# ikryukov/svo

Hardware: AMD Instinct MI355X
Metric: frames/sec @1241x376, 2000 feats; LK iters/sec; achieved HBM GB/s (higher is better)
Workload: dtype u8/int32 fixed-point (LK sums exact int, solve f32), f64 PnP

## Files before the change

svo_amd/csrc/lk_device.hpp:

```cpp
#pragma once
#include "common.hpp"

#include <cfloat>
#include <cmath>

namespace svo {

namespace {

constexpr int W_BITS = 14;
constexpr float FLT_SCALE = 1.f / (1 << 20);
constexpr int JM = 3;

struct LKDev {
    int win_w, win_h, groups;
    int ip_w, ip_h, jr_w, jr_h;
    int ip_bytes, lds_wave;
    int max_level, max_count;
    double eps2;
    float eps2_lo, eps2_hi;
    int flags, want_err;
    float min_eig;
};

inline LKDev lk_dev(const LKParams& lp) {
    LKDev d;
    d.win_w = lp.win_w;
    d.win_h = lp.win_h;
    d.groups = 64 / lp.win_w;
    d.ip_w = lp.win_w;
    d.ip_h = lp.win_h + 1;
    d.jr_w = lp.win_w + 2 * JM;
    d.jr_h = lp.win_h + 1 + 2 * JM;
    d.ip_bytes = (d.ip_w * d.ip_h * 4 + 15) & ~15;
    d.lds_wave = d.ip_bytes + ((d.jr_w * d.jr_h * 4 + 15) & ~15);
    d.max_level = lp.max_level;
    d.max_count = lp.max_count;
    d.eps2 = lp.eps2;
    d.eps2_lo = (float)(lp.eps2 * (1.0 - 0x1p-20));
    d.eps2_hi = (float)(lp.eps2 * (1.0 + 0x1p-20));
    if ((double)d.eps2_lo > lp.eps2 * (1.0 - 0x1p-20)) d.eps2_lo = nextafterf(d.eps2_lo, 0.f);
    if ((double)d.eps2_hi < lp.eps2 * (1.0 + 0x1p-20)) d.eps2_hi = nextafterf(d.eps2_hi, INFINITY);
    d.flags = lp.flags;
    d.want_err = lp.want_err;
    d.min_eig = lp.min_eig;
    return d;
}

__device__ __forceinline__ bool converged(float dx, float dy, float lo, float hi, double eps2) {
    const float sf = dx * dx + dy * dy;
    bool c = sf < lo;
    if (__builtin_expect(sf >= lo && sf <= hi, 0)) {
        asm volatile("" ::: "memory");
        c = (double)dx * dx + (double)dy * dy <= eps2;
    }
    return c;
}
__device__ __forceinline__ bool below_001(float v) { return fabsf(v) <= 0x1.47ae14p-7f; }

__device__ __forceinline__ int refl101(int p, int len) {
    if ((unsigned)p < (unsigned)len) return p;
    if (len == 1) return 0;
    do {
        p = p < 0 ? -p : 2 * len - 2 - p;
    } while ((unsigned)p >= (unsigned)len);
    return p;
}

__device__ __forceinline__ int ufloor(float v) {
    return (int)__builtin_floorf(v);
}
__device__ __forceinline__ float uni_f(float v) {
    return __int_as_float(__builtin_amdgcn_readfirstlane(__float_as_int(v)));
}
__device__ __forceinline__ int uni_i(int v) { return __builtin_amdgcn_readfirstlane(v); }

__device__ __forceinline__ void wave_lds_sync() {
    __builtin_amdgcn_fence(__ATOMIC_SEQ_CST, "wavefront");
    __builtin_amdgcn_wave_barrier();
}

__device__ __forceinline__ int dpp_sum(int v) {
    v += __builtin_amdgcn_update_dpp(0, v, 0xb1, 0xf, 0xf, true);
    v += __builtin_amdgcn_update_dpp(0, v, 0x4e, 0xf, 0xf, true);
    v += __builtin_amdgcn_update_dpp(0, v, 0x114, 0xf, 0xf, true);
    v += __builtin_amdgcn_update_dpp(0, v, 0x118, 0xf, 0xf, true);
    v += __builtin_amdgcn_update_dpp(0, v, 0x142, 0xa, 0xf, true);
    v += __builtin_amdgcn_update_dpp(0, v, 0x143, 0xc, 0xf, true);
    return __builtin_amdgcn_readlane(v, 63);
}
__device__ __forceinline__ double wave_sum_exact(int v) {
    int hi = dpp_sum(v >> 16);
    int lo = dpp_sum(v & 0xFFFF);
    return (double)((long long)hi * 65536 + (long long)lo);
}
template <int CTRL, int ROW_MASK, bool BC>
__device__ __forceinline__ int dpp_add(int v) {
    return v + __builtin_amdgcn_update_dpp(0, v, CTRL, ROW_MASK, 0xf, BC);
}

typedef const __attribute__((address_space(1))) uint8_t* gu8;
typedef const __attribute__((address_space(1))) uint32_t* gu32;
typedef short s16x2 __attribute__((ext_vector_type(2)));
typedef uint32_t u32x2a4 __attribute__((ext_vector_type(2), aligned(4)));
typedef uint16_t u16a1 __attribute__((aligned(1)));
typedef const __attribute__((address_space(4))) PyrDesc* cpyr;

template <typename T>
__device__ __forceinline__ T ldg_off(gu8 base, unsigned off) {
    return *(const __attribute__((address_space(1))) T*)(base + off);
}
__device__ __forceinline__ gu8 pad_origin(const uint8_t* data, int pitch, int pad_px, int elem) {
    return (gu8)data - (size_t)pad_px * ((size_t)pitch + 1) * elem;
}

__device__ __forceinline__ int sdot2(unsigned a, unsigned b, int c) {
    return __builtin_amdgcn_sdot2(__builtin_bit_cast(s16x2, a), __builtin_bit_cast(s16x2, b), c, false);
}
__device__ __forceinline__ int sdot2_r(unsigned a, unsigned b, int c) {
    int d;
    asm("v_dot2_i32_i16 %0, %1, %2, %3" : "=v"(d) : "v"(a), "v"(b), "v"(c));
    return d;
}
__device__ __forceinline__ unsigned lo16x2(int lo, int hi) {
    return __builtin_amdgcn_perm((unsigned)hi, (unsigned)lo, 0x05040100u);
}

__device__ __forceinline__ unsigned wbits(float p) { return __float_as_uint(p + 768.f); }
struct BiW {
    unsigned W0, W1;
};
__device__ __forceinline__ BiW bilinear_weights(float a, float b) {
    const float ia = 1.f - a, ib = 1.f - b;
    const unsigned b00 = wbits(ia * ib), b01 = wbits(a * ib), b10 = wbits(ia * b);
    const unsigned w11 = (1u << W_BITS) + 3u * 0x44400000u - b00 - b01 - b10;
    return {__builtin_amdgcn_perm(b01, b00, 0x05040100u), __builtin_amdgcn_perm(w11, b10, 0x05040100u)};
}

struct SubPix {
    int ix, iy;
    BiW w;
};
__device__ __forceinline__ SubPix sub_pixel(float x, float y) {
    const float fx = __builtin_floorf(x), fy = __builtin_floorf(y);
    return {(int)fx, (int)fy, bilinear_weights(x - fx, y - fy)};
}
__device__ __forceinline__ bool window_in_bounds(int x, int y, int w, int h, int win_w, int win_h) {
    return (unsigned)(x + win_w) < (unsigned)(w + win_w) && (unsigned)(y + win_h) < (unsigned)(h + win_h);
}

struct LevelStart {
    float nextx, nexty;
    int ipx, ipy;
    bool inb;
    float a, b;
};
__device__ __forceinline__ LevelStart level_start(float px, float py, float nx, float ny, int level, int max_level,
                                                  int flags, int lw, int lh, int win_w, int win_h) {
    const float halfWx = (win_w - 1) * 0.5f, halfWy = (win_h - 1) * 0.5f;
    const float lscale = __builtin_amdgcn_ldexpf(1.f, -level);
    float prevx = px * lscale, prevy = py * lscale;
    float nextx, nexty;
    if (level == max_level) {
        if (flags & SVO_LK_USE_INITIAL_FLOW) {
            nextx = nx * lscale;
            nexty = ny * lscale;
        } else {
            nextx = prevx;
            nexty = prevy;
        }
    } else {
        nextx = nx * 2.f;
        nexty = ny * 2.f;
    }
    prevx -= halfWx;
    prevy -= halfWy;
    const float fpx = __builtin_floorf(prevx), fpy = __builtin_floorf(prevy);
    const int ipx = (int)fpx, ipy = (int)fpy;
    return {nextx, nexty, ipx, ipy, window_in_bounds(ipx, ipy, lw, lh, win_w, win_h), prevx - fpx, prevy - fpy};
}

template <int M, class Stage>
__device__ __forceinline__ void follow_region(int x, int y, int& jx0, int& jy0, Stage stage) {
    if ((unsigned)(x - jx0) > 2u * M || (unsigned)(y - jy0) > 2u * M) {
        jx0 = x - M;
        jy0 = y - M;
        wave_lds_sync();
        stage();
        wave_lds_sync();
    }
}

template <int M, class Stage, class RowSad>
__device__ __forceinline__ bool sad_error(float nx, float ny, int jw, int jh, int win_w, int win_h, int& jx0,
                                          int& jy0, Stage stage, RowSad row_sad, float& errv) {
    const SubPix s = sub_pixel(nx - (win_w - 1) * 0.5f, ny - (win_h - 1) * 0.5f);
    const int ix0 = uni_i(s.ix), iy0 = uni_i(s.iy);
    if (!window_in_bounds(ix0, iy0, jw, jh, win_w, win_h)) return false;
    follow_region<M>(ix0, iy0, jx0, jy0, stage);
    errv = (float)wave_sum_exact(row_sad(ix0, iy0, s.w)) * 1.f / (float)(32 * win_w * win_h);
    return true;
}

__device__ __forceinline__ void store_track(const LKBatch& B, float* next_xy, size_t base, int pt, float nx,
                                            float ny, int st, float errv, int itcount) {
    next_xy[2 * pt] = nx;
    next_xy[2 * pt + 1] = ny;
    B.status[base + pt] = (uint8_t)st;
    if (B.err) B.err[base + pt] = errv;
    if (B.iters) B.iters[base + pt] = itcount;
}

}

hipError_t launch_lk_multi_temporal(const LKBatch& b, int nseq, int max_n, const LKParams& lp, hipStream_t st);
hipError_t launch_lk_multi_stereo(const LKBatch& b, int nseq, int max_n, const LKParams& lp, hipStream_t st);
hipError_t launch_lk_cvq(const LKBatch& b, int nseq, int max_n, const LKParams& lp, hipStream_t st);
hipError_t launch_lk_fast(const LKBatch& b, int nseq, int max_n, const LKParams& lp, hipStream_t st);
hipError_t launch_lk_generic(const LKBatch& b, int nseq, int max_n, const LKParams& lp, hipStream_t st);
hipError_t launch_lk_cv(const LKBatch& b, int nseq, int max_n, const LKParams& lp, hipStream_t st);

}
```

svo_amd/csrc/lk_multi.hip:

```cpp
#include "lk_quad.hpp"
#include "xcd_tile.hpp"

namespace svo {

namespace {

__device__ __forceinline__ unsigned hi16x2(int lo, int hi) {
    return __builtin_amdgcn_perm((unsigned)hi, (unsigned)lo, 0x07060302u);
}
__device__ __forceinline__ int swz16_add(int v) {
    return v + __builtin_amdgcn_ds_swizzle(v, 0x401f);
}
__device__ __forceinline__ float halves_lane_float(int h, int l) { return __builtin_fmaf((float)h, 65536.f, (float)l); }

__device__ __forceinline__ void pair_setup(unsigned I2, unsigned GXm, unsigned GYm, int& a11, int& a12, int& a22,
                                           int& c1, int& c2) {
    a11 = sdot2(GXm, GXm, a11);
    a12 = sdot2(GXm, GYm, a12);
    a22 = sdot2(GYm, GYm, a22);
    c1 = sdot2(I2, GXm, c1);
    c2 = sdot2(I2, GYm, c2);
}
template <int NR, bool ODD>
__device__ __forceinline__ void strip_setup_c(const unsigned* P, const u32x2a4* D, unsigned IW0, unsigned IW1,
                                              unsigned GW0, unsigned GW1, unsigned* GX, unsigned* GY, int& a11,
                                              int& a12, int& a22, int& c1, int& c2, int& li, int& lx, int& ly) {
    constexpr int NP = ODD ? NR / 2 : (NR + 1) / 2;
    const int rnd_i = 1 << (W_BITS - 6), rnd_d = 1 << (W_BITS + kDerShift - 1);
    int iv[NR + 1], gx[NR + 1], gy[NR + 1];
    iv[NR] = gx[NR] = gy[NR] = 0;
#pragma unroll
    for (int j = 0; j < NR; j++) {
        iv[j] = sdot2(P[j], IW0, sdot2_r(P[j + 1], IW1, rnd_i)) >> (W_BITS - 5);
        const unsigned X0 = __builtin_amdgcn_perm(D[j].y, D[j].x, 0x05040100u);
        const unsigned X1 = __builtin_amdgcn_perm(D[j + 1].y, D[j + 1].x, 0x05040100u);
        const unsigned Y0 = __builtin_amdgcn_perm(D[j].y, D[j].x, 0x07060302u);
        const unsigned Y1 = __builtin_amdgcn_perm(D[j + 1].y, D[j + 1].x, 0x07060302u);
        gx[j] = sdot2(X0, GW0, sdot2_r(X1, GW1, rnd_d));
        gy[j] = sdot2(Y0, GW0, sdot2_r(Y1, GW1, rnd_d));
    }
    static_assert(W_BITS + kDerShift == 16, "derivative sums must carry their descaled value in bits 16..31");
#pragma unroll
    for (int m = 0; m < NP; m++) {
        GX[m] = hi16x2(gx[2 * m], gx[2 * m + 1]);
        GY[m] = hi16x2(gy[2 * m], gy[2 * m + 1]);
        pair_setup(lo16x2(iv[2 * m], iv[2 * m + 1]), GX[m], GY[m], a11, a12, a22, c1, c2);
    }
    if constexpr (ODD) {
        li = iv[NR - 1];
        lx = gx[NR - 1];
        ly = gy[NR - 1];
    }
}
__device__ __forceinline__ void odd_pair_setup(int i0, int x0, int y0, int i1, int x1, int y1, unsigned& GXm,
                                               unsigned& GYm, int& a11, int& a12, int& a22, int& c1, int& c2) {
    GXm = hi16x2(x0, x1);
    GYm = hi16x2(y0, y1);
    pair_setup(lo16x2(i0, i1), GXm, GYm, a11, a12, a22, c1, c2);
}

template <int LPF, int STEPS32>
__device__ __forceinline__ int group_add_step(int v, int step) {
    switch (step) {
        case 0: return dpp_row_add<0xb1>(v);
        case 1: return dpp_row_add<0x4e>(v);
        case 2: return dpp_row_add<0x124>(v);
        case 3: return dpp_row_add<0x128>(v);
        default: return swz16_add(v);
    }
}
template <int LPF, int STEPS32, int NV>
__device__ __forceinline__ void group_sum_f(int (&v)[NV], float (&f)[NV]) {
    constexpr int STEPS = LPF == 16 ? 4 : 5;
    static_assert(LPF == 16 || LPF == 32, "groups of 16 or 32 lanes");
#pragma unroll
    for (int s = 0; s < STEPS32; s++)
#pragma unroll
        for (int i = 0; i < NV; i++) v[i] = group_add_step<LPF, STEPS32>(v[i], s);
    int h[NV], lo[NV];
#pragma unroll
    for (int i = 0; i < NV; i++) {
        h[i] = v[i] >> 16;
        lo[i] = v[i] & 0xFFFF;
    }
#pragma unroll
    for (int s = STEPS32; s < STEPS; s++)
#pragma unroll
        for (int i = 0; i < NV; i++) {
            h[i] = group_add_step<LPF, STEPS32>(h[i], s);
            lo[i] = group_add_step<LPF, STEPS32>(lo[i], s);
        }
#pragma unroll
    for (int i = 0; i < NV; i++) f[i] = halves_lane_float(h[i], lo[i]);
}
template <int LPF, int STEPS32>
__device__ __forceinline__ void group_halves(int v, int& h, int& lo) {
    constexpr int STEPS = LPF == 16 ? 4 : 5;
#pragma unroll
    for (int s = 0; s < STEPS32; s++) v = group_add_step<LPF, STEPS32>(v, s);
    h = v >> 16;
    lo = v & 0xFFFF;
#pragma unroll
    for (int s = STEPS32; s < STEPS; s++) {
        h = group_add_step<LPF, STEPS32>(h, s);
        lo = group_add_step<LPF, STEPS32>(lo, s);
    }
}
__device__ __forceinline__ void wave_halves2(int x, int y, int& xh, int& xl, int& yh, int& yl) {
    x = dpp_add<0xb1, 0xf, true>(x);
    y = dpp_add<0xb1, 0xf, true>(y);
    x = dpp_add<0x4e, 0xf, true>(x);
    y = dpp_add<0x4e, 0xf, true>(y);
    x = dpp_add<0x114, 0xf, true>(x);
    y = dpp_add<0x114, 0xf, true>(y);
    int ah = x >> 16, al = x & 0xFFFF, bh = y >> 16, bl = y & 0xFFFF;
    ah = dpp_add<0x118, 0xf, true>(ah);
    al = dpp_add<0x118, 0xf, true>(al);
    bh = dpp_add<0x118, 0xf, true>(bh);
    bl = dpp_add<0x118, 0xf, true>(bl);
    ah = dpp_add<0x142, 0xa, false>(ah);
    al = dpp_add<0x142, 0xa, false>(al);
    bh = dpp_add<0x142, 0xa, false>(bh);
    bl = dpp_add<0x142, 0xa, false>(bl);
    ah = dpp_add<0x143, 0xc, false>(ah);
    al = dpp_add<0x143, 0xc, false>(al);
    bh = dpp_add<0x143, 0xc, false>(bh);
    bl = dpp_add<0x143, 0xc, false>(bl);
    xh = __builtin_amdgcn_readlane(ah, 63);
    xl = __builtin_amdgcn_readlane(al, 63);
    yh = __builtin_amdgcn_readlane(bh, 63);
    yl = __builtin_amdgcn_readlane(bl, 63);
}
__device__ __forceinline__ float rl_f(float v, int lane) {
    return __int_as_float(__builtin_amdgcn_readlane(__float_as_int(v), lane));
}

template <int FPW, int QJM, int MINW, int KKS = 2, int WW = 21, int WH = 21, int NR = 7, bool LOOP = false>
__global__ __launch_bounds__(64, MINW) void lk_multi_kernel(LKBatch B, LKDev p) {
    using Q = MultiShape<QJM, WW, WH, FPW>;
    static_assert(WH % NR == 0, "whole strips");
    static_assert(WW + QJM + 3 <= kPyrPad && WW + 1 <= kDerPad, "padding too small for the window");
    constexpr int JRW = Q::JRW, JRH = Q::JRH;
    constexpr int NSTRIP = WW * (WH / NR);
    constexpr int LPF = 64 / FPW;
    constexpr int K = (NSTRIP + LPF - 1) / LPF;
    constexpr bool ODD = NR % 2 == 1 && K % 2 == 0;
    constexpr int NP = ODD ? NR / 2 : (NR + 1) / 2;
    constexpr int NO = ODD ? K / 2 : 1;
    constexpr long long kProd = (long long)NR * K * 8160 * 4080;
    constexpr int STEPS32 = 4 * kProd < (1ll << 31) ? 2 : 2 * kProd < (1ll << 31) ? 1 : 0;
    static_assert(kProd < (1ll << 31), "a lane's partial sums must fit int32");
    constexpr bool TAIL = !LOOP && FPW == 4 && K == 4 && ODD && NP == 3 && NO == 2;
    static_assert(!TAIL || 8ll * (2 * NP + 2) * 8160 * 4080 < (1ll << 31), "tail partials: 3 int32 DPP steps");
    extern __shared__ __attribute__((aligned(16))) uint8_t lds[];
    const int lane = threadIdx.x & 63;
    const int g = lane / LPF, l = lane % LPF;
    const XcdTile tile = xcd_tile();
    const int seq = tile.y;
    const int n = B.counts ? B.counts[seq] : B.n;
    int tx = tile.x;
next_tile:
    const int pt0 = tx * FPW;
    if (pt0 >= n) return;
    const int pt = pt0 + g;
    const bool live = pt < n;
    const int ptc = live ? pt : n - 1;
    const size_t base = (size_t)seq * B.cap;
    const float* __restrict__ prev_xy = B.prev_xy + 2 * base;
    float* __restrict__ next_xy = B.next_xy + 2 * base;
    const cpyr prev = (cpyr)B.prev + seq;
    const cpyr next = (cpyr)B.next + seq;
    const DerivDesc& dprev = B.dprev[seq];
    unsigned* jregs = reinterpret_cast<unsigned*>(lds);
    const unsigned* jmine = jregs + g * (Q::JSTRIDE / 4);
    const StageGeom<JRW, JRH> sg(lane);

    int scol[K], srow[K];
    bool sreal[K];
#pragma unroll
    for (int k = 0; k < K; k++) {
        const int sidx = l + LPF * k;
        sreal[k] = sidx < NSTRIP;
        const int sc = sreal[k] ? sidx : 0;
        scol[k] = sc % WW;
        srow[k] = (sc / WW) * NR;
    }
    constexpr float halfWx = (WW - 1) * 0.5f, halfWy = (WH - 1) * 0.5f;
    const int rnd_j = 1 << (W_BITS - 6 + kJShift);

    const float px = prev_xy[2 * ptc], py = prev_xy[2 * ptc + 1];
    float nx = 0.f, ny = 0.f;
    if (p.flags & SVO_LK_USE_INITIAL_FLOW) {
        nx = next_xy[2 * ptc];
        ny = next_xy[2 * ptc + 1];
    }
    int st = live ? 1 : 0;
    float errv = 0.f;
    int itc[FPW];
#pragma unroll
    for (int f = 0; f < FPW; f++) itc[f] = 0;
    const int max_level = p.max_level;

    for (int level = max_level; level >= 0; level--) {
        const ImgLevel I{prev->lv[level].data, prev->lv[level].w, prev->lv[level].h, prev->lv[level].pitch};
        const ImgLevel J{next->lv[level].data, next->lv[level].w, next->lv[level].h, next->lv[level].pitch};
        const LevelStart start = level_start(px, py, nx, ny, level, max_level, p.flags, I.w, I.h, WW, WH);
        float nextx = start.nextx, nexty = start.nexty;
        nx = nextx;
        ny = nexty;
        const int ipx = start.ipx, ipy = start.ipy;
        const bool inb = start.inb;
        if (!inb && level == 0 && live) {
            st = 0;
            errv = 0.f;
        }
        bool lact = live && inb;
        const BiW iw = bilinear_weights(start.a, start.b);
        const unsigned IW0 = iw.W0, IW1 = iw.W1;

        int jx0 = ufloor(nextx - halfWx) - QJM, jy0 = ufloor(nexty - halfWy) - QJM;
        int jxa = jx0 & ~3;
        int jbase = jy0 * JRW + jxa;
        unsigned GX[K][NP], GY[K][NP], GXO[NO], GYO[NO];
        int li[K], lx[K], ly[K];
        int asum[3] = {0, 0, 0};
        int csum[2] = {0, 0};
        {
            using SL = StageGeom<JRW, JRH>;
            int xs[FPW], ys[FPW];
#pragma unroll
            for (int f = 0; f < FPW; f++) {
                const int xa = __builtin_amdgcn_readlane(jxa, LPF * f), y0 = __builtin_amdgcn_readlane(jy0, LPF * f);
                const bool ok = __builtin_amdgcn_readlane((int)lact, LPF * f) && region_in_pad<JRW, JRH>(J, xa, y0);
                xs[f] = ok ? xa : 0;
                ys[f] = ok ? y0 : 0;
            }
            unsigned sv[FPW][SL::NPS];
            const gu8 jbase = pad_origin(J.data, J.pitch, kPyrPad, 1) + (size_t)kPyrPad * (J.pitch + 1);
            const unsigned ol = 4u * (unsigned)sg.d + (unsigned)sg.row(0) * (unsigned)J.pitch;
            const unsigned olast = 4u * (unsigned)sg.d + (unsigned)sg.row(SL::NPS - 1) * (unsigned)J.pitch;
#pragma unroll
            for (int f = 0; f < FPW; f++) {
                const gu8 fb = jbase + xs[f] + (ptrdiff_t)ys[f] * J.pitch;
#pragma unroll
                for (int q = 0; q < SL::NPS; q++)
                    sv[f][q] = q + 1 < SL::NPS ? ldg_off<unsigned>(fb + (size_t)q * SL::RPP * J.pitch, ol)
                                               : ldg_off<unsigned>(fb, olast);
            }
            const int dpitch = dprev.pitch[level];
            const gu8 ibase = pad_origin(I.data, I.pitch, kPyrPad, 1);
            const gu8 dbase = pad_origin((const uint8_t*)dprev.data[level], dpitch, kDerPad, 4);
            const int sx = inb ? ipx : 0, sy = inb ? ipy : 0;
            const auto load_strip = [&](int k, unsigned* P, u32x2a4* Dv) {
                const int x = sx + scol[k], y = sy + srow[k];
                const unsigned oi = (unsigned)(x + kPyrPad) + (unsigned)(y + kPyrPad) * (unsigned)I.pitch;
                const unsigned od = 4u * ((unsigned)(x + kDerPad) + (unsigned)(y + kDerPad) * (unsigned)dpitch);
#pragma unroll
                for (int r = 0; r <= NR; r++) {
                    P[r] = __builtin_amdgcn_perm(0u, (unsigned)ldg_off<u16a1>(ibase + (size_t)r * I.pitch, oi),
                                                 0x0c010c00u);
                    Dv[r] = ldg_off<u32x2a4>(dbase + (size_t)r * 4 * dpitch, od);
                }
            };
            const auto write_staging = [&] {
#pragma unroll
                for (int f = 0; f < FPW; f++)
#pragma unroll
                    for (int q = 0; q < SL::NPS; q++) sg.write(jregs + f * (Q::JSTRIDE / 4), sg.row(q), sv[f][q]);
            };
            static_assert(KKS >= 1, "strips loaded per setup group");
#pragma unroll
            for (int k0 = 0; k0 < K; k0 += KKS) {
                constexpr int KK = K >= KKS ? KKS : 1;
                unsigned P[KK][NR + 1];
                u32x2a4 Dv[KK][NR + 1];
#pragma unroll
                for (int kk = 0; kk < KK; kk++) load_strip(k0 + kk, P[kk], Dv[kk]);
                if (k0 == 0) write_staging();
#pragma unroll
                for (int kk = 0; kk < KK; kk++) {
                    const int k = k0 + kk;
                    strip_setup_c<NR, ODD>(P[kk], Dv[kk], IW0, IW1, sreal[k] ? IW0 : 0u, sreal[k] ? IW1 : 0u, GX[k],
                                           GY[k], asum[0], asum[1], asum[2], csum[0], csum[1], li[k], lx[k], ly[k]);
                    if (ODD && (k & 1))
                        odd_pair_setup(li[k - 1], lx[k - 1], ly[k - 1], li[k], lx[k], ly[k], GXO[k / 2], GYO[k / 2],
                                       asum[0], asum[1], asum[2], csum[0], csum[1]);
                }
            }
        }
        wave_lds_sync();
        float A[3];
        group_sum_f<LPF, STEPS32>(asum, A);
        const float A11 = A[0] * FLT_SCALE, A12 = A[1] * FLT_SCALE, A22 = A[2] * FLT_SCALE;

        float D = A11 * A22 - A12 * A12;
        const float minEig =
            (A22 + A11 - sqrtf((A11 - A22) * (A11 - A22) + 4.f * A12 * A12)) / (float)(2 * WW * WH);
        if (lact && p.want_err && (p.flags & SVO_LK_GET_MIN_EIGENVALS)) errv = minEig;
        if (lact && (minEig < p.min_eig || D < FLT_EPSILON)) {
            if (level == 0) st = 0;
            lact = false;
        }
        D = 1.f / D;
        const float Ds = D * FLT_SCALE;

        nextx -= halfWx;
        nexty -= halfWy;
        float pdx = 0.f, pdy = 0.f;
        int tail_j = -1;
        for (int j = 0; j < p.max_count; j++) {
            const unsigned long long act0 = __builtin_amdgcn_ballot_w64(lact);
            if (act0 == 0) break;
            if constexpr (TAIL) {
                const unsigned long long gm = act0 & 0x0001000100010001ull;
                if ((gm & (gm - 1)) == 0) {
                    tail_j = j;
                    break;
                }
            }
            const float fnx = __builtin_floorf(nextx), fny = __builtin_floorf(nexty);
            const int inx = (int)fnx, iny = (int)fny;
            if (lact && !window_in_bounds(inx, iny, J.w, J.h, WW, WH)) {
                if (level == 0) st = 0;
                lact = false;
            }
            const bool need = lact && ((unsigned)(inx - jx0) > 2u * QJM || (unsigned)(iny - jy0) > 2u * QJM);
            unsigned long long nb = __builtin_amdgcn_ballot_w64(need && l == 0);
            if (nb) {
                if (need) {
                    jx0 = inx - QJM;
                    jy0 = iny - QJM;
                    jxa = jx0 & ~3;
                    jbase = jy0 * JRW + jxa;
                }
                wave_lds_sync();
                while (nb) {
                    const int f = (int)(__builtin_ctzll(nb) / LPF);
                    nb &= nb - 1;
                    stage_padded<JRW, JRH>(jregs + f * (Q::JSTRIDE / 4), J,
                                           __builtin_amdgcn_readlane(jxa, LPF * f),
                                           __builtin_amdgcn_readlane(jy0, LPF * f), sg);
                }
                wave_lds_sync();
            }
            {
                const unsigned long long act = __builtin_amdgcn_ballot_w64(lact);
#pragma unroll
                for (int f = 0; f < FPW; f++) itc[f] += (int)((act >> (LPF * f)) & 1ull);
            }
            const BiW w = bilinear_weights(nextx - fnx, nexty - fny);
            const unsigned W0 = w.W0, W1 = w.W1;
            int bsum[2] = {-csum[0], -csum[1]};
            {
                const int off = lact ? __mul24(iny, JRW) + inx - jbase : 0;
                const unsigned* jb = jmine + off;
                int jlast = 0;
#pragma unroll
                for (int k = 0; k < K; k++) {
                    const unsigned* js = jb + srow[k] * JRW + scol[k];
                    unsigned q[NR + 1];
#pragma unroll
                    for (int r = 0; r <= NR; r++) q[r] = js[r * JRW];
                    int jv[NR + 1];
                    jv[NR] = 0;
#pragma unroll
                    for (int r = 0; r < NR; r++)
                        jv[r] = sdot2(q[r], W0, sdot2_r(q[r + 1], W1, rnd_j));
#pragma unroll
                    for (int m = 0; m < NP; m++) {
                        const unsigned jj = hi16x2(jv[2 * m], jv[2 * m + 1]);
                        bsum[0] = sdot2(jj, GX[k][m], bsum[0]);
                        bsum[1] = sdot2(jj, GY[k][m], bsum[1]);
                    }
                    if constexpr (ODD) {
                        if (k & 1) {
                            const unsigned jj = hi16x2(jlast, jv[NR - 1]);
                            bsum[0] = sdot2(jj, GXO[k / 2], bsum[0]);
                            bsum[1] = sdot2(jj, GYO[k / 2], bsum[1]);
                        } else {
                            jlast = jv[NR - 1];
                        }
                    }
                }
            }
            float fb[2];
            group_sum_f<LPF, STEPS32>(bsum, fb);
            asm volatile("" : "+v"(fb[0]), "+v"(fb[1]));
            const float fb1 = fb[0], fb2 = fb[1];
            const float dx = (A12 * fb2 - A22 * fb1) * Ds;
            const float dy = (A12 * fb1 - A11 * fb2) * Ds;
            if (lact) {
                nextx += dx;
                nexty += dy;
                nx = nextx + halfWx;
                ny = nexty + halfWy;
                if (converged(dx, dy, p.eps2_lo, p.eps2_hi, p.eps2)) {
                    lact = false;
                } else if (j > 0 && below_001(dx + pdx) && below_001(dy + pdy)) {
                    nx -= dx * 0.5f;
                    ny -= dy * 0.5f;
                    lact = false;
                } else {
                    pdx = dx;
                    pdy = dy;
                }
            }
        }
        if constexpr (TAIL) {
            if (tail_j >= 0) {
                const int fs = (int)(__builtin_ctzll(__builtin_amdgcn_ballot_w64(lact)) / LPF);
                const int ls = fs * LPF;
                unsigned* const gst = jregs + ((fs + 1) & (FPW - 1)) * (Q::JSTRIDE / 4);
                unsigned* const jstar = jregs + fs * (Q::JSTRIDE / 4);
                if (g == fs) {
#pragma unroll
                    for (int k = 0; k < K; k++) {
                        const int t = ((k >> 1) << 5) | (l << 1) | (k & 1);
                        const unsigned ox = (k & 1) ? GXO[k >> 1] : 0u, oy = (k & 1) ? GYO[k >> 1] : 0u;
                        *reinterpret_cast<uint4*>(gst + 8 * t) = uint4{GX[k][0], GX[k][1], GX[k][2], GY[k][0]};
                        *reinterpret_cast<uint4*>(gst + 8 * t + 4) = uint4{GY[k][1], GY[k][2], ox, oy};
                    }
                }
                int ch0, cl0, ch1, cl1;
                group_halves<LPF, STEPS32>(csum[0], ch0, cl0);
                group_halves<LPF, STEPS32>(csum[1], ch1, cl1);
                ch0 = __builtin_amdgcn_readlane(ch0, ls);
                cl0 = __builtin_amdgcn_readlane(cl0, ls);
                ch1 = __builtin_amdgcn_readlane(ch1, ls);
                cl1 = __builtin_amdgcn_readlane(cl1, ls);
                wave_lds_sync();
                const uint4 ga = *reinterpret_cast<const uint4*>(gst + 8 * lane);
                const uint4 gb = *reinterpret_cast<const uint4*>(gst + 8 * lane + 4);
                const unsigned TX[NP] = {ga.x, ga.y, ga.z}, TY[NP] = {ga.w, gb.x, gb.y};
                const unsigned TXO = gb.z, TYO = gb.w;
                int soff;
                {
                    const int sidx = ((lane >> 1) & (LPF - 1)) + LPF * (((lane >> 5) << 1) | (lane & 1));
                    const int sc = sidx < NSTRIP ? sidx : 0;
                    soff = (sc / WW) * NR * JRW + sc % WW;
                }
                float tnx = rl_f(nextx, ls), tny = rl_f(nexty, ls), tpdx = rl_f(pdx, ls), tpdy = rl_f(pdy, ls);
                float tox = rl_f(nx, ls), toy = rl_f(ny, ls);
                const float tA11 = rl_f(A11, ls), tA12 = rl_f(A12, ls), tA22 = rl_f(A22, ls), tDs = rl_f(Ds, ls);
                int tjx0 = __builtin_amdgcn_readlane(jx0, ls), tjy0 = __builtin_amdgcn_readlane(jy0, ls);
                int tjbase = __builtin_amdgcn_readlane(jbase, ls);
                int tst = __builtin_amdgcn_readlane(st, ls);
                int titc = 0;
                for (int j = tail_j; j < p.max_count; j++) {
                    const float fnx = __builtin_floorf(tnx), fny = __builtin_floorf(tny);
                    const int inx = (int)fnx, iny = (int)fny;
                    if (!window_in_bounds(inx, iny, J.w, J.h, WW, WH)) {
                        if (level == 0) tst = 0;
                        break;
                    }
                    if ((unsigned)(inx - tjx0) > 2u * QJM || (unsigned)(iny - tjy0) > 2u * QJM) {
                        tjx0 = inx - QJM;
                        tjy0 = iny - QJM;
                        tjbase = tjy0 * JRW + (tjx0 & ~3);
                        wave_lds_sync();
                        stage_padded<JRW, JRH>(jstar, J, tjx0 & ~3, tjy0, sg);
                        wave_lds_sync();
                    }
                    titc++;
                    const BiW w = bilinear_weights(tnx - fnx, tny - fny);
                    const unsigned* js = jstar + (__mul24(iny, JRW) + inx - tjbase) + soff;
                    unsigned q[NR + 1];
#pragma unroll
                    for (int r = 0; r <= NR; r++) q[r] = js[r * JRW];
                    int jv[NR];
#pragma unroll
                    for (int r = 0; r < NR; r++) jv[r] = sdot2(q[r], w.W0, sdot2_r(q[r + 1], w.W1, rnd_j));
                    int b0 = 0, b1 = 0;
#pragma unroll
                    for (int m = 0; m < NP; m++) {
                        const unsigned jj = hi16x2(jv[2 * m], jv[2 * m + 1]);
                        b0 = sdot2(jj, TX[m], b0);
                        b1 = sdot2(jj, TY[m], b1);
                    }
                    {
                        const int jp = __builtin_amdgcn_update_dpp(0, jv[NR - 1], 0xb1, 0xf, 0xf, true);
                        const unsigned jj = hi16x2(jp, jv[NR - 1]);
                        b0 = sdot2(jj, TXO, b0);
                        b1 = sdot2(jj, TYO, b1);
                    }
                    int h0, l0, h1, l1;
                    wave_halves2(b0, b1, h0, l0, h1, l1);
                    const float fb1 = __builtin_fmaf((float)(h0 - ch0), 65536.f, (float)(l0 - cl0));
                    const float fb2 = __builtin_fmaf((float)(h1 - ch1), 65536.f, (float)(l1 - cl1));
                    const float dx = (tA12 * fb2 - tA22 * fb1) * tDs;
                    const float dy = (tA12 * fb1 - tA11 * fb2) * tDs;
                    tnx += dx;
                    tny += dy;
                    tox = tnx + halfWx;
                    toy = tny + halfWy;
                    if (converged(dx, dy, p.eps2_lo, p.eps2_hi, p.eps2)) break;
                    if (j > 0 && below_001(dx + tpdx) && below_001(dy + tpdy)) {
                        tox -= dx * 0.5f;
                        toy -= dy * 0.5f;
                        break;
                    }
                    tpdx = dx;
                    tpdy = dy;
                }
                if (g == fs) {
                    nx = tox;
                    ny = toy;
                    st = tst;
                }
#pragma unroll
                for (int f = 0; f < FPW; f++) itc[f] += f == fs ? titc : 0;
            }
        }
        wave_lds_sync();
    }
    if (l == 0 && live) {
        next_xy[2 * pt] = nx;
        next_xy[2 * pt + 1] = ny;
        B.status[base + pt] = (uint8_t)st;
        if (B.err) B.err[base + pt] = errv;
        if (B.iters) {
            int itcount = itc[0];
#pragma unroll
            for (int f = 1; f < FPW; f++) itcount = g == f ? itc[f] : itcount;
            B.iters[base + pt] = itcount;
        }
    }
    if constexpr (LOOP) {
        tx += gridDim.x;
        goto next_tile;
    }
}

template <int FPW, int QJM, int MINW, int KKS, int WW, int WH, int NR, bool LOOP>
hipError_t launch_multi(const LKBatch& b, int nseq, int max_n, const LKParams& lp, hipStream_t st) {
    const int gn = LOOP && b.grid_hint > 0 && b.grid_hint < max_n ? b.grid_hint : max_n;
    dim3 grid((gn + FPW - 1) / FPW, nseq);
    constexpr int lds_bytes = FPW * MultiShape<QJM, WW, WH, FPW>::JSTRIDE;
    hipLaunchKernelGGL((lk_multi_kernel<FPW, QJM, MINW, KKS, WW, WH, NR, LOOP>), grid, dim3(64), lds_bytes, st, b,
                       lk_dev(lp));
    return hipGetLastError();
}

}

hipError_t launch_lk_multi_temporal(const LKBatch& b, int nseq, int max_n, const LKParams& lp, hipStream_t st) {
    return launch_multi<4, 1, 3, 2, 21, 21, 7, false>(b, nseq, max_n, lp, st);
}

hipError_t launch_lk_multi_stereo(const LKBatch& b, int nseq, int max_n, const LKParams& lp, hipStream_t st) {
    return launch_multi<4, 1, 6, 1, 11, 11, 11, true>(b, nseq, max_n, lp, st);
}

}
```

Baseline: 117,000.

## Remap LK strips so each lane loads three adjacent strips in one wide load

```diff
diff --git a/svo_amd/csrc/lk_device.hpp b/svo_amd/csrc/lk_device.hpp
--- a/svo_amd/csrc/lk_device.hpp
+++ b/svo_amd/csrc/lk_device.hpp
@@ -103,7 +103,9 @@
 typedef const __attribute__((address_space(1))) uint32_t* gu32;
 typedef short s16x2 __attribute__((ext_vector_type(2)));
 typedef uint32_t u32x2a4 __attribute__((ext_vector_type(2), aligned(4)));
+typedef uint32_t u32x4a4 __attribute__((ext_vector_type(4), aligned(4)));
 typedef uint16_t u16a1 __attribute__((aligned(1)));
+typedef uint32_t u32a1 __attribute__((aligned(1)));
 typedef const __attribute__((address_space(4))) PyrDesc* cpyr;
 
 template <typename T>
diff --git a/svo_amd/csrc/lk_multi.hip b/svo_amd/csrc/lk_multi.hip
--- a/svo_amd/csrc/lk_multi.hip
+++ b/svo_amd/csrc/lk_multi.hip
@@ -1,4 +1,5 @@
 #include "lk_quad.hpp"
+#include "lk_strip_map.hpp"
 #include "xcd_tile.hpp"
 
 namespace svo {
@@ -144,6 +145,12 @@
     constexpr int NSTRIP = WW * (WH / NR);
     constexpr int LPF = 64 / FPW;
     constexpr int K = (NSTRIP + LPF - 1) / LPF;
+    using SM = StripMap<WW, WH / NR, LPF>;
+    static_assert(SM::K == K && SM::valid(), "strip map");
+    constexpr bool TRI = SM::TRIPLES;
+    static_assert(!TRI || K == 4, "a triple and a single per lane");
+    static_assert(WW + 1 <= kPyrPad && WH + 1 <= kPyrPad && WW + 1 <= kDerPad && WH + 1 <= kDerPad,
+                  "padding too small for the prev window's loads");
     constexpr bool ODD = NR % 2 == 1 && K % 2 == 0;
     constexpr int NP = ODD ? NR / 2 : (NR + 1) / 2;
     constexpr int NO = ODD ? K / 2 : 1;
@@ -179,11 +186,10 @@
     bool sreal[K];
 #pragma unroll
     for (int k = 0; k < K; k++) {
-        const int sidx = l + LPF * k;
-        sreal[k] = sidx < NSTRIP;
-        const int sc = sreal[k] ? sidx : 0;
-        scol[k] = sc % WW;
-        srow[k] = (sc / WW) * NR;
+        const Strip s = SM::at(l, k);
+        sreal[k] = s.real;
+        scol[k] = s.col;
+        srow[k] = s.band * NR;
     }
     constexpr float halfWx = (WW - 1) * 0.5f, halfWy = (WH - 1) * 0.5f;
     const int rnd_j = 1 << (W_BITS - 6 + kJShift);
@@ -251,6 +257,12 @@
             const gu8 ibase = pad_origin(I.data, I.pitch, kPyrPad, 1);
             const gu8 dbase = pad_origin((const uint8_t*)dprev.data[level], dpitch, kDerPad, 4);
             const int sx = inb ? ipx : 0, sy = inb ? ipy : 0;
+            const auto write_staging = [&] {
+#pragma unroll
+                for (int f = 0; f < FPW; f++)
+#pragma unroll
+                    for (int q = 0; q < SL::NPS; q++) sg.write(jregs + f * (Q::JSTRIDE / 4), sg.row(q), sv[f][q]);
+            };
             const auto load_strip = [&](int k, unsigned* P, u32x2a4* Dv) {
                 const int x = sx + scol[k], y = sy + srow[k];
                 const unsigned oi = (unsigned)(x + kPyrPad) + (unsigned)(y + kPyrPad) * (unsigned)I.pitch;
@@ -262,29 +274,54 @@
                     Dv[r] = ldg_off<u32x2a4>(dbase + (size_t)r * 4 * dpitch, od);
                 }
             };
-            const auto write_staging = [&] {
-#pragma unroll
-                for (int f = 0; f < FPW; f++)
-#pragma unroll
-                    for (int q = 0; q < SL::NPS; q++) sg.write(jregs + f * (Q::JSTRIDE / 4), sg.row(q), sv[f][q]);
+            const auto setup_strip = [&](int k, const unsigned* P, const u32x2a4* Dv) {
+                strip_setup_c<NR, ODD>(P, Dv, IW0, IW1, sreal[k] ? IW0 : 0u, sreal[k] ? IW1 : 0u, GX[k], GY[k], asum[0],
+                                       asum[1], asum[2], csum[0], csum[1], li[k], lx[k], ly[k]);
+                if (ODD && (k & 1))
+                    odd_pair_setup(li[k - 1], lx[k - 1], ly[k - 1], li[k], lx[k], ly[k], GXO[k / 2], GYO[k / 2],
+                                   asum[0], asum[1], asum[2], csum[0], csum[1]);
             };
-            static_assert(KKS >= 1, "strips loaded per setup group");
-#pragma unroll
-            for (int k0 = 0; k0 < K; k0 += KKS) {
-                constexpr int KK = K >= KKS ? KKS : 1;
-                unsigned P[KK][NR + 1];
-                u32x2a4 Dv[KK][NR + 1];
-#pragma unroll
-                for (int kk = 0; kk < KK; kk++) load_strip(k0 + kk, P[kk], Dv[kk]);
-                if (k0 == 0) write_staging();
-#pragma unroll
-                for (int kk = 0; kk < KK; kk++) {
-                    const int k = k0 + kk;
-                    strip_setup_c<NR, ODD>(P[kk], Dv[kk], IW0, IW1, sreal[k] ? IW0 : 0u, sreal[k] ? IW1 : 0u, GX[k],
-                                           GY[k], asum[0], asum[1], asum[2], csum[0], csum[1], li[k], lx[k], ly[k]);
-                    if (ODD && (k & 1))
-                        odd_pair_setup(li[k - 1], lx[k - 1], ly[k - 1], li[k], lx[k], ly[k], GXO[k / 2], GYO[k / 2],
-                                       asum[0], asum[1], asum[2], csum[0], csum[1]);
+            if constexpr (TRI) {
+                unsigned M[NR + 1];
+                u32x4a4 Dm[NR + 1];
+                {
+                    const int x = sx + scol[0], y = sy + srow[0];
+                    const unsigned oi = (unsigned)(x + kPyrPad) + (unsigned)(y + kPyrPad) * (unsigned)I.pitch;
+                    const unsigned od = 4u * ((unsigned)(x + kDerPad) + (unsigned)(y + kDerPad) * (unsigned)dpitch);
+#pragma unroll
+                    for (int r = 0; r <= NR; r++) {
+                        M[r] = ldg_off<u32a1>(ibase + (size_t)r * I.pitch, oi);
+                        Dm[r] = ldg_off<u32x4a4>(dbase + (size_t)r * 4 * dpitch, od);
+                    }
+                }
+                write_staging();
+                unsigned P[NR + 1], Ps[NR + 1];
+                u32x2a4 Dv[NR + 1], Ds[NR + 1];
+#pragma unroll
+                for (int k = 0; k < 3; k++) {
+                    if (k == 2) load_strip(3, Ps, Ds);
+#pragma unroll
+                    for (int r = 0; r <= NR; r++) {
+                        P[r] = __builtin_amdgcn_perm(0u, M[r], k == 0 ? 0x0c010c00u : k == 1 ? 0x0c020c01u : 0x0c030c02u);
+                        Dv[r] = k == 0   ? u32x2a4{Dm[r].x, Dm[r].y}
+                                : k == 1 ? u32x2a4{Dm[r].y, Dm[r].z}
+                                         : u32x2a4{Dm[r].z, Dm[r].w};
+                    }
+                    setup_strip(k, P, Dv);
+                }
+                setup_strip(3, Ps, Ds);
+            } else {
+                static_assert(KKS >= 1, "strips loaded per setup group");
+#pragma unroll
+                for (int k0 = 0; k0 < K; k0 += KKS) {
+                    constexpr int KK = K >= KKS ? KKS : 1;
+                    unsigned P[KK][NR + 1];
+                    u32x2a4 Dv[KK][NR + 1];
+#pragma unroll
+                    for (int kk = 0; kk < KK; kk++) load_strip(k0 + kk, P[kk], Dv[kk]);
+                    if (k0 == 0) write_staging();
+#pragma unroll
+                    for (int kk = 0; kk < KK; kk++) setup_strip(k0 + kk, P[kk], Dv[kk]);
                 }
             }
         }
@@ -435,9 +472,8 @@
                 const unsigned TXO = gb.z, TYO = gb.w;
                 int soff;
                 {
-                    const int sidx = ((lane >> 1) & (LPF - 1)) + LPF * (((lane >> 5) << 1) | (lane & 1));
-                    const int sc = sidx < NSTRIP ? sidx : 0;
-                    soff = (sc / WW) * NR * JRW + sc % WW;
+                    const Strip s = SM::at((lane >> 1) & (LPF - 1), ((lane >> 5) << 1) | (lane & 1));
+                    soff = s.band * NR * JRW + s.col;
                 }
                 float tnx = rl_f(nextx, ls), tny = rl_f(nexty, ls), tpdx = rl_f(pdx, ls), tpdy = rl_f(pdy, ls);
                 float tox = rl_f(nx, ls), toy = rl_f(ny, ls);
diff --git a/svo_amd/csrc/lk_strip_map.hpp b/svo_amd/csrc/lk_strip_map.hpp
--- /dev/null
+++ b/svo_amd/csrc/lk_strip_map.hpp
@@ -0,0 +1,71 @@
+#pragma once
+
+namespace svo {
+
+struct Strip {
+    int col, band;
+    bool real;
+};
+
+template <int WW, int NB, int LPF>
+struct StripMap {
+    static constexpr int NSTRIP = WW * NB;
+    static constexpr int K = (NSTRIP + LPF - 1) / LPF;
+    static constexpr bool TRIPLES = WW == 21 && NB == 3 && LPF == 16;
+
+    static constexpr Strip at(int l, int k) {
+        if constexpr (TRIPLES) {
+            if (k < 3) {
+                const int band = (l >= 5 ? 1 : 0) + (l >= 10 ? 1 : 0);
+                return {3 * (l - 5 * band) + (band == 2 ? 3 : 0) + k, band, true};
+            }
+            const int band = (l >= 6 ? 1 : 0) + (l >= 12 ? 1 : 0);
+            return {l == 15 ? 0 : band == 2 ? l - 12 : 15 + l - 6 * band, l == 15 ? 0 : band, l != 15};
+        } else {
+            const int sidx = l + LPF * k;
+            const bool real = sidx < NSTRIP;
+            const int sc = real ? sidx : 0;
+            return {sc % WW, sc / WW, real};
+        }
+    }
+
+    static constexpr bool valid() {
+        int seen[NSTRIP] = {};
+        int dummies = 0;
+        for (int l = 0; l < LPF; l++)
+            for (int k = 0; k < K; k++) {
+                const Strip s = at(l, k);
+                if (s.col < 0 || s.col >= WW || s.band < 0 || s.band >= NB) return false;
+                if (s.real)
+                    seen[s.band * WW + s.col]++;
+                else
+                    dummies++;
+                if (TRIPLES && k < 3) {
+                    const Strip a = at(l, 0);
+                    if (!s.real || s.col != a.col + k || s.band != a.band) return false;
+                }
+            }
+        for (int i = 0; i < NSTRIP; i++)
+            if (seen[i] != 1) return false;
+        return dummies == LPF * K - NSTRIP;
+    }
+    static constexpr bool bank_free(int JRW, int NR) {
+        for (int k = 0; k < K; k++) {
+            bool used[32] = {};
+            for (int l = 0; l < LPF; l++) {
+                const Strip s = at(l, k);
+                const int b = (s.band * NR * JRW + s.col) % 32;
+                if (used[b]) return false;
+                used[b] = true;
+            }
+        }
+        return true;
+    }
+};
+
+static_assert(StripMap<21, 3, 16>::TRIPLES && StripMap<21, 3, 16>::K == 4 && StripMap<21, 3, 16>::valid(),
+              "21 x 21: 16 triples, 15 singles, 1 dummy");
+static_assert(StripMap<21, 3, 16>::bank_free(26, 7), "21 x 21, 1-px margin: a slot's lanes on 16 banks");
+static_assert(!StripMap<11, 1, 16>::TRIPLES && StripMap<11, 1, 16>::valid(), "11 x 11: one strip per lane");
+
+}
```

Result: faster. 120,600 (median of 6 runs) (+3.1%).
